# cosmodesi/cosmoprimo

Hardware: AMD Instinct MI355X
Metric: batched FFTLog P(k)->xi(r) transforms/sec (N=2048) (higher is better)
Workload: dtype f64; 1 GPU; config 2: 100000 rows x N_k=2048 per GPU, PowerToCorrelation(ell=0), Np=4096, extrap=0; rows_per_gpu=100000, n_k=2048, padded_size=4096, parallelism=rows sharded over 1 GPU(s), no collective, grid=512, block=256, lds_bytes=69936, rccl_ranks=0

## Files before the change

### cosmoprimo_amd/_lib.py

```python
import ctypes
import os

import numpy as np

_HERE = os.path.dirname(os.path.abspath(__file__))
LIB_PATH = os.path.join(_HERE, 'libcosmoprimo_amd.so')
ABI_VERSION = 4

CP_OK, CP_EINVAL, CP_EUNSUPPORTED, CP_EDEVICE, CP_ENOMEM = range(5)
EXTRAP_CONSTANT, EXTRAP_EDGE, EXTRAP_LOGLOG = range(3)
(KERNEL_BESSEL_J, KERNEL_SPHERICAL_BESSEL_J, KERNEL_TOPHAT, KERNEL_TOPHAT_SQ, KERNEL_GAUSSIAN, KERNEL_GAUSSIAN_SQ) = range(6)
KERNEL_CUSTOM = 100


class FFTlogSpec(ctypes.Structure):
    _fields_ = [('kind', ctypes.c_int), ('param', ctypes.c_double), ('q', ctypes.c_double), ('xy', ctypes.c_double), ('pre_power', ctypes.c_double),
                ('pre_const', ctypes.c_double), ('post_sign', ctypes.c_double)]


_c_double_p = ctypes.POINTER(ctypes.c_double)
_c_int_p = ctypes.POINTER(ctypes.c_int)

SIGNATURES = {
    'cp_abi_version': (ctypes.c_int, []),
# ... 1 lines not shown
    'cp_device_count': (ctypes.c_int, []),
    'cp_loggamma': (ctypes.c_int, [_c_double_p, _c_double_p, ctypes.c_longlong]),
    'cp_gamma': (ctypes.c_int, [_c_double_p, _c_double_p, ctypes.c_longlong]),
    'cp_kernel_eval': (ctypes.c_int, [ctypes.c_int, ctypes.c_double, _c_double_p, _c_double_p, ctypes.c_longlong]),
    'cp_fftlog_padded_size': (ctypes.c_int, [ctypes.c_int, ctypes.c_int]),
    'cp_fftlog_tables': (ctypes.c_int, [ctypes.c_int, ctypes.c_int, _c_double_p, ctypes.POINTER(FFTlogSpec), ctypes.c_int, ctypes.c_int, ctypes.c_int,
                                       _c_double_p, _c_double_p] + [_c_double_p] * 8),
    'cp_fftlog_plan_create': (ctypes.c_int, [ctypes.POINTER(ctypes.c_void_p), ctypes.c_int, ctypes.c_int, ctypes.c_int, _c_double_p,
                                            _c_double_p, _c_double_p, ctypes.c_int]),
    'cp_fftlog_execute': (ctypes.c_int, [ctypes.c_void_p, ctypes.c_void_p, ctypes.c_void_p, ctypes.c_longlong, ctypes.c_int, ctypes.c_double,
                                        ctypes.c_int, ctypes.c_double, ctypes.c_int, ctypes.c_void_p]),
    'cp_fftlog_execute_window': (ctypes.c_int, [ctypes.c_void_p, ctypes.c_void_p, ctypes.c_void_p, ctypes.c_longlong, ctypes.c_int, ctypes.c_double,
                                               ctypes.c_int, ctypes.c_double, ctypes.c_int, ctypes.c_int, ctypes.c_int, ctypes.c_void_p]),
    'cp_fftlog_plan_destroy': (ctypes.c_int, [ctypes.c_void_p]),
    'cp_fftlog_plan_info': (ctypes.c_int, [ctypes.c_void_p, ctypes.c_longlong, _c_int_p, _c_int_p, _c_int_p]),
    'cp_background_distance': (ctypes.c_int, [ctypes.c_longlong, ctypes.c_longlong, ctypes.c_void_p, ctypes.c_int, ctypes.c_void_p, ctypes.c_int,
                                             ctypes.c_void_p, ctypes.c_int, ctypes.c_int, ctypes.c_void_p]),
    'cp_derived_parameters': (ctypes.c_int, [ctypes.c_longlong, ctypes.c_void_p, ctypes.c_void_p, ctypes.c_int, ctypes.c_void_p]),
    'cp_background_knots': (ctypes.c_int, [_c_double_p, ctypes.c_int]),
    'cp_background_init': (ctypes.c_int, [ctypes.c_int]),
    'cp_distance_from_radial': (ctypes.c_int, [ctypes.c_void_p, ctypes.c_void_p, ctypes.c_longlong, ctypes.c_double, ctypes.c_int, ctypes.c_void_p, ctypes.c_int, ctypes.c_void_p]),
    'cp_ncdm_knots': (ctypes.c_int, [_c_double_p, ctypes.c_int]),
    'cp_growth_ode_knots': (ctypes.c_int, [_c_double_p, ctypes.c_int]),
    'cp_growth_ode_tables': (ctypes.c_int, [ctypes.c_longlong, ctypes.c_void_p, ctypes.c_int, ctypes.c_void_p, ctypes.c_int, ctypes.c_void_p, ctypes.c_int,
                                           ctypes.c_void_p]),
    'cp_ncdm_tables': None,
    'cp_background_eval': (ctypes.c_int, [ctypes.c_longlong, ctypes.c_longlong, ctypes.c_void_p, ctypes.c_int, ctypes.c_void_p, ctypes.c_void_p,
                                         ctypes.c_int, ctypes.c_void_p, ctypes.c_int, ctypes.c_int, ctypes.c_void_p]),
    'cp_power_workspace_bytes': (ctypes.c_longlong, [ctypes.c_longlong]),
    'cp_power_eval': (ctypes.c_int, [ctypes.c_int, ctypes.c_int, ctypes.c_longlong, ctypes.c_void_p, ctypes.c_int, ctypes.c_void_p, ctypes.c_void_p,
# ... 265 lines not shown
```

### cosmoprimo_amd/csrc/cp_fftlog.hip

```cpp
#include <hip/hip_runtime.h>

#include <cstring>
#include <new>
#include <vector>

#include "../../include/cosmoprimo_amd.h"
#include "cp_error.h"
#include "cp_fftlog_kernel.h"
#include "cp_fftlog_large.h"
#include "cp_internal.h"

using namespace cpfft;

namespace {

bool find_launcher(int npad, Launcher* out) {
    return find_launcher_g0(npad, out) || find_launcher_g1(npad, out) || find_launcher_g2(npad, out) || find_launcher_g3(npad, out) ||
           find_launcher_g4(npad, out);
}

}

struct cp_fftlog_plan {
    int n, npad, nker, device;
    int in_left, out_left;
    Launcher l;
    int max_grid[VAR_COUNT];
    double* d_pre;
    double* d_post;
    cplx* d_u;
    cplx* d_tw;
    unsigned* d_ticket;
    cp_fftlog_large* large;
};

#define CP_HIP(call)                                                                               \
    do {                                                                                           \
        hipError_t e_ = (call);                                                                    \
        if (e_ != hipSuccess) {                                                                    \
            status = cp::fail(e_ == hipErrorOutOfMemory ? CP_ENOMEM : CP_EDEVICE, "%s: %s", #call, hipGetErrorString(e_)); \
            goto done;                                                                             \
        }                                                                                          \
    } while (0)

bool cp_fftlog_plan_view(const cp_fftlog_plan* p, cp_fftlog_tables_view* out) {
    if (!p || p->large || !out) return false;
    *out = cp_fftlog_tables_view{p->n, p->npad, p->nker, p->device, p->in_left, p->out_left, p->d_pre, p->d_post, p->d_u, p->d_tw};
    return true;
}
// ... 17 lines not shown
    if (npad < n || (npad & (npad - 1)) != 0)
        return cp::fail(CP_EINVAL, "cp_fftlog_plan_create: padded size %d must be a power of two >= n=%d (fftlog.py:149-159)", npad, n);
    Launcher l;
    if (npad > (1 << 24)) return cp::fail(CP_EUNSUPPORTED, "cp_fftlog_plan_create: padded size %d is beyond the supported range (2^24)", npad);
    if ((long long)nker * npad > (1LL << 28))
        return cp::fail(CP_EUNSUPPORTED, "cp_fftlog_plan_create: %d transforms of padded size %d: tables of more than 2^28 entries", nker, npad);
    if (npad > CP_FFTLOG_MAX_NP) {
        cp_fftlog_plan* p = new (std::nothrow) cp_fftlog_plan();
        if (!p) return cp::fail(CP_ENOMEM, "cp_fftlog_plan_create: host allocation failed");
        p->n = n; p->npad = npad; p->nker = nker; p->device = device;
        p->in_left = (npad - n) / 2;
        p->out_left = (npad - n) - (npad - n) / 2;
        p->d_pre = p->d_post = nullptr;
        p->d_u = p->d_tw = nullptr;
        p->d_ticket = nullptr;
        p->large = nullptr;
        cp::DeviceScope scope(device);
        int st = scope.ok() ? cp_fftlog_large_create(&p->large, n, npad, nker, pre, post, u_re_im, device)
                          : cp::fail(CP_EDEVICE, "cp_fftlog_plan_create: cannot select device %d", device);
        if (st != CP_OK) {
            delete p;
            return st;
        }
        *out = p;
        return CP_OK;
    }
    if (!find_launcher(npad, &l))
        return cp::fail(CP_EUNSUPPORTED, "cp_fftlog_plan_create: padded size %d outside the LDS-resident kernel range [4, %d]", npad,
                        CP_FFTLOG_MAX_NP);
    int status = CP_OK;
    cp_fftlog_plan* p = new (std::nothrow) cp_fftlog_plan();
    if (!p) return cp::fail(CP_ENOMEM, "cp_fftlog_plan_create: host allocation failed");
    p->large = nullptr;
    p->n = n;
    p->npad = npad;
    p->nker = nker;
    p->device = device;
    p->in_left = (npad - n) / 2;
    p->out_left = (npad - n) - (npad - n) / 2;
    p->l = l;
    p->d_pre = p->d_post = nullptr;
    p->d_u = p->d_tw = nullptr;
    p->d_ticket = nullptr;
    {
        cp::DeviceScope scope(device);
        std::vector<cplx> tw, u((size_t)nker * npad);
        if (!scope.ok()) {
            status = cp::fail(CP_EDEVICE, "cp_fftlog_plan_create: cannot select device %d", device);
            goto done;
        }
        l.build_tw(tw);
        for (int k = 0; k < nker; ++k) l.build_u(u_re_im + (size_t)k * 2 * (npad / 2 + 1), u.data() + (size_t)k * npad);
        const size_t tbytes = (size_t)nker * npad * sizeof(double);
        CP_HIP(hipMalloc(&p->d_pre, tbytes));
        CP_HIP(hipMalloc(&p->d_post, tbytes));
        CP_HIP(hipMalloc(&p->d_u, u.size() * sizeof(cplx)));
        CP_HIP(hipMalloc(&p->d_tw, tw.size() * sizeof(cplx)));
        CP_HIP(hipMemcpy(p->d_pre, pre, tbytes, hipMemcpyHostToDevice));
        CP_HIP(hipMemcpy(p->d_post, post, tbytes, hipMemcpyHostToDevice));
        CP_HIP(hipMemcpy(p->d_u, u.data(), u.size() * sizeof(cplx), hipMemcpyHostToDevice));
        CP_HIP(hipMemcpy(p->d_tw, tw.data(), tw.size() * sizeof(cplx), hipMemcpyHostToDevice));
        CP_HIP(hipMalloc(&p->d_ticket, CP_CU_SLOTS * sizeof(unsigned)));
        CP_HIP(hipMemset(p->d_ticket, 0, CP_CU_SLOTS * sizeof(unsigned)));
        int ncu = 0;
        CP_HIP(hipDeviceGetAttribute(&ncu, hipDeviceAttributeMultiprocessorCount, device));
        for (int v = 0; v < VAR_COUNT; ++v) {
            p->max_grid[v] = 0;
            if (!l.func[v]) continue;
            const int lds_v = l.lds_bytes + l.lds_extra[v];
            if (lds_v > 64 * 1024) CP_HIP(hipFuncSetAttribute(l.func[v], hipFuncAttributeMaxDynamicSharedMemorySize, lds_v));
            int nblk = 0;
            CP_HIP(hipOccupancyMaxActiveBlocksPerMultiprocessor(&nblk, l.func[v], l.block, lds_v));
            if (nblk < 1) {
                status = cp::fail(CP_EDEVICE, "cp_fftlog_plan_create: kernel variant %d for npad=%d does not fit on a CU", v, npad);
                goto done;
            }
            p->max_grid[v] = nblk * ncu;
        }
// ... 4 lines not shown
        return status;
    }
    *out = p;
    return CP_OK;
}

extern "C" int cp_fftlog_plan_destroy(cp_fftlog_plan* p) {
    if (!p) return CP_OK;
    {
        cp::DeviceScope scope(p->device);
        if (p->d_pre) (void)hipFree(p->d_pre);
        if (p->d_post) (void)hipFree(p->d_post);
        if (p->d_u) (void)hipFree(p->d_u);
        if (p->d_tw) (void)hipFree(p->d_tw);
        if (p->d_ticket) (void)hipFree(p->d_ticket);
        cp_fftlog_large_destroy(p->large);
    }
    delete p;
    return CP_OK;
}

static int grid_for(const cp_fftlog_plan* p, int variant, long long nbatch) {
    const long long npairs = ((nbatch + 1) / 2) * p->nker;
    return (int)(npairs < p->max_grid[variant] ? npairs : p->max_grid[variant]);
}

extern "C" int cp_fftlog_plan_info(const cp_fftlog_plan* p, long long nbatch, int* grid, int* block, int* lds_bytes) {
    if (!p) return cp::fail(CP_EINVAL, "cp_fftlog_plan_info: null plan");
    if (p->large) {
        if (grid) *grid = 0;
        if (block) *block = 0;
        if (lds_bytes) *lds_bytes = 0;
        return CP_OK;
    }
    const int variant = select_variant(p->npad, p->l.p, p->n, 0, 0., 0, 0., 0);
    if (grid) *grid = grid_for(p, variant, nbatch);
    if (block) *block = p->l.block;
    if (lds_bytes) *lds_bytes = p->l.lds_bytes + p->l.lds_extra[variant];
    return CP_OK;
}

static int execute_impl(const cp_fftlog_plan* p, const double* d_in, double* d_out, long long nbatch, int extrap_left, double val_left, int extrap_right,
                        double val_right, int keep_padding, int out_first, int out_count, void* stream) {
    if (!p) return cp::fail(CP_EINVAL, "cp_fftlog_execute: null plan");
    if (nbatch < 0) return cp::fail(CP_EINVAL, "cp_fftlog_execute: negative batch");
    if (nbatch == 0) return CP_OK;
    if (!d_in || !d_out) return cp::fail(CP_EINVAL, "cp_fftlog_execute: null device pointer");
    if (extrap_left < CP_EXTRAP_CONSTANT || extrap_left > CP_EXTRAP_LOGLOG || extrap_right < CP_EXTRAP_CONSTANT || extrap_right > CP_EXTRAP_LOGLOG)
        return cp::fail(CP_EINVAL, "cp_fftlog_execute: unknown extrapolation mode (%d, %d)", extrap_left, extrap_right);
    if (p->large) {
        cp::DeviceScope scope(p->device);
        if (!scope.ok()) return cp::fail(CP_EDEVICE, "cp_fftlog_execute: cannot select device %d", p->device);
        return cp_fftlog_large_execute(p->large, d_in, d_out, nbatch, extrap_left, val_left, extrap_right, val_right, keep_padding,
// ... 20 lines not shown
    A.cu_ticket = p->d_ticket;
    A.out_first = 0;
    A.out_last = A.n_out;
    cp::DeviceScope scope(p->device);
    if (!scope.ok()) return cp::fail(CP_EDEVICE, "cp_fftlog_execute: cannot select device %d", p->device);
    int variant = select_variant(p->npad, p->l.p, p->n, extrap_left, val_left, extrap_right, val_right, keep_padding);
    if (variant == VAR_HALF_ZERO && out_count >= 0 && out_count < A.n_out && p->l.func[VAR_HALF_ZERO_WINDOW]) {
        variant = VAR_HALF_ZERO_WINDOW;
        A.out_first = out_first;
        A.out_last = out_first + out_count;
        A.stream_rows = (double)nbatch * p->nker * ((double)p->n + out_count) * 8. > 512. * 1024. * 1024. ? 3 : 0;
    }
    const int grid = grid_for(p, variant, nbatch);
    if ((long long)p->nker * p->npad >= (1LL << 31) || 2LL * grid * p->npad >= (1LL << 31))
        return cp::fail(CP_EUNSUPPORTED, "cp_fftlog_execute: nker = %d kernels of padded size %d exceed the row-walk range", p->nker, p->npad);
    p->l.launch(variant, A, grid, static_cast<hipStream_t>(stream));
    return cp::launch_status("cp_fftlog_execute");
}

extern "C" int cp_fftlog_execute(const cp_fftlog_plan* p, const double* d_in, double* d_out, long long nbatch, int extrap_left,
                                 double val_left, int extrap_right, double val_right, int keep_padding, void* stream) {
    return execute_impl(p, d_in, d_out, nbatch, extrap_left, val_left, extrap_right, val_right, keep_padding, 0, -1, stream);
}

extern "C" int cp_fftlog_execute_window(const cp_fftlog_plan* p, const double* d_in, double* d_out, long long nbatch, int extrap_left, double val_left,
                                        int extrap_right, double val_right, int keep_padding, int out_first, int out_count, void* stream) {
    if (p) {
        const int n_out = keep_padding ? p->npad : p->n;
        if (out_first < 0 || out_count < 0 || out_first > n_out - out_count)
            return cp::fail(CP_EINVAL, "cp_fftlog_execute_window: columns [%d, %d + %d) are not inside the %d of an output row", out_first, out_first, out_count, n_out);
// ... 4 lines not shown
```

### cosmoprimo_amd/csrc/cp_fftlog_body.h

```cpp
#pragma once
#include <math.h>

#include "cp_fft_core.h"
#if defined(__HIPCC__)
#include "cp_math.h"
#endif

namespace cpfft {

enum { CP_EXTRAP_CONST = 0, CP_EXTRAP_EDGE = 1, CP_EXTRAP_LOG = 2 };

#ifndef CP_INTERPAIR_BARRIER
#define CP_INTERPAIR_BARRIER 0
#endif
#ifndef CP_WAVE_SKEW
#define CP_WAVE_SKEW 1
#endif
#ifndef CP_WAVE_ORDER
#define CP_WAVE_ORDER 0x3210
#endif
#ifndef CP_WIDE_IO
#define CP_WIDE_IO 0
#endif
#ifndef CP_ROW_SCREEN
// ... 21 lines not shown
    long long nbatch;
    int nker;
    int n;
    int in_left;
    int out_off;
    int n_out;
    int ext_l, ext_r;
    double val_l, val_r;
    int stream_rows;
    const double* pre;
    const double* post;
    const cplx* u;
    const cplx* tw;
    int out_first, out_last;
    unsigned* cu_ticket;
#if defined(CP_STAMPS)
    double* val_stamp;
    unsigned long long* bar_log;
    int bar_log_pairs;
#endif
};

template <int NP, int P, int IN_MODE = IN_LOG, int OUT_MODE = OUT_GENERIC>
struct Fftlog {
    using PL = Plan<NP, P>;
    static constexpr int T = PL::T;
    static constexpr int NPASS = PL::NPASS;
    static constexpr int NPH = 2 * NPASS - 1;
    static constexpr int LAST = NPASS - 1;
    static constexpr bool EARLY_TW1 = CP_EARLY_TW1 && NPASS >= 3 && CP_ABLATE == 0;
// ... 407 lines not shown
                const int o = nidx - A.out_off;
                if (o >= 0 && o < A.n_out) {
                    const double f = post[nidx];
                    double ya = x[s].re * f, yb = x[s].im * f;
                    if constexpr (SCREEN) fix_output<1>(fix, &ya, &yb);
                    oa[o] = ya;
                    if (has_b) ob[o] = yb;
                }
            }
        }
    }

    struct State {
        int t0;
        unsigned info_cur, info_nxt;
        cplx w[P];
        cplx wpin[KPIN > 0 ? KPIN : 1];
        double fpre[H], fpost[H];
        double va[H], vb[H];
#if defined(CP_STAMPS)
        unsigned long long fs[8], fs_last;
#endif
    };

    template <int I>
    static CP_HD void load_twiddles(int t, const FftlogArgs& A, cplx* w) {
        Pass<NP, P, I>::template twiddle_load<(I == 0 ? KPIN : 0)>(t, A.tw + PL::tw_offset(I), w);
    }
    template <class ST>
    static CP_HD void merge_pinned(const ST& st, cplx* wl) {
// ... 40 lines not shown
            }
#pragma unroll
            for (int r = 0; r < H; ++r) {
                st.va[r] *= st.fpre[r];
                st.vb[r] *= st.fpre[r];
            }
            unsigned ma = 0, mb = 0;
            thread_max<H>(st.va, st.vb, ma, mb);
            screen_publish(t, lds, ma, mb);
        }
#endif
    }

    static CP_HD void init_state(int t, const FftlogArgs& A, const double* ra, const double* rb, int ker, State& st) {
        st.t0 = pass0_thread(t);
        if constexpr (NPASS > 1) load_twiddles<0>(st.t0, A, st.w);
        if constexpr (KPIN > 0) {
            const cplx* tw0 = A.tw + PL::tw_offset(0);
#pragma unroll
            for (int s = 1; s <= KPIN; ++s) st.wpin[s - 1] = ld_cplx(tw0, (unsigned)st.t0 * 16u, (unsigned)(s * T) * 16u);
        }
        if constexpr (HALF_IN) {
            load_factors_half(st.t0, A, ker, st);
            if constexpr (ROWS_FROM_MEMORY) prefetch_rows(st.t0, ra, rb, st.va, st.vb, A.stream_rows);
        }
    }

    template <int PHN>
    static CP_HD void load_tables_for(int t, int t0, const FftlogArgs& A, int ker, cplx* w) {
        if constexpr (PHN == LAST) {
// ... 33 lines not shown
        if constexpr (NPASS == 1) {
            load_input(t0, t, A, ra, rb, has_b, pre, lds, st.info_cur, x);
            Pass<NP, P, 0>::butterflies(x);
            load_u(t0, A, ker, st.w);
            mul_w(st.w, x);
            Pass<NP, P, 0>::butterflies(x);
            store_output(t0, A, oa, ob, has_b, post, st.info_cur, x);
        } else if constexpr (PH == 0) {
            if constexpr (HALF_IN) {
#if defined(__HIP_DEVICE_COMPILE__)
                if constexpr (SCREEN_AHEAD) st.info_cur = gate(st.info_nxt);
#endif
                load_input_half(t0, t, A, ra, rb, has_b, pre, lds, st, x);
                CP_SCHED_FENCE();
                if constexpr (ROWS_FROM_MEMORY) prefetch_rows(t0, nra, nrb, st.va, st.vb, A.stream_rows);
                CP_SCHED_FENCE();
            } else {
                load_input(t0, t, A, ra, rb, has_b, pre, lds, st.info_cur, x);
            }
            if constexpr (KPIN > 0) {
                cplx wl[P];
                merge_pinned(st, wl);
                Pass<NP, P, 0>::template butterflies_store<ZERO_PADDED_IN, true>(t0, wl, lds, x);
            } else {
                Pass<NP, P, 0>::template butterflies_store<ZERO_PADDED_IN, true>(t0, st.w, lds, x);
            }
            load_tables_for<1>(t, t0, A, ker, st.w);
            if constexpr (EARLY_TW1) Pass<NP, P, 1>::twiddle_load_lds(t, lds_tw<1>(lds), st.w);
        } else if constexpr (PH < LAST) {
            constexpr int I = (PH < LAST) ? PH : 0;
// ... 60 lines not shown
```

### cosmoprimo_amd/csrc/cp_fftlog_dispatch.h

```cpp
#pragma once

#ifdef CP_FFTLOG_ONLY
#define CP_FFTLOG_SIZES(X) X(CP_FFTLOG_ONLY, 16)
#else
#define CP_FFTLOG_SIZES(X) \
    X(4, 4)                \
    X(8, 8)                \
    X(16, 16)              \
    X(32, 16)              \
    X(64, 16)              \
    X(128, 16)             \
    X(256, 16)             \
    X(512, 16)             \
    X(1024, 16)            \
    X(2048, 16)            \
    X(4096, 16)            \
    X(8192, 16)
#endif

#define CP_FFTLOG_MAX_NP 8192

enum { VAR_GENERIC = 0, VAR_LOG = 1, VAR_HALF = 2, VAR_HALF_ZERO = 3, VAR_HALF_ZERO_WINDOW = 4, VAR_COUNT = 5 };

#define CP_FFTLOG_HALF_MIN_NP 512

inline int select_variant(int np, int p, int n, int ext_l, double val_l, int ext_r, double val_r, int keep_padding) {
    if (ext_l == 2 || ext_r == 2) return VAR_LOG;
    if ((p == 16 || p == 8) && np >= CP_FFTLOG_HALF_MIN_NP && 2 * n == np && !keep_padding) {
        if (ext_l == 0 && ext_r == 0 && val_l == 0. && val_r == 0.) return VAR_HALF_ZERO;
        return VAR_HALF;
    }
    return VAR_GENERIC;
}
```

### cosmoprimo_amd/csrc/cp_fftlog_kernel.h

```cpp
#pragma once
#include <hip/hip_runtime.h>

#include <vector>

#include "cp_fftlog_body.h"
#include "cp_fftlog_dispatch.h"
#include "cp_fftlog_tables.h"

namespace cpfft {

struct Launcher {
    const void* func[VAR_COUNT];
    void (*launch)(int variant, const FftlogArgs&, int grid, hipStream_t stream);
    int np, p, block, lds_bytes;
    int lds_extra[VAR_COUNT];
    void (*build_tw)(std::vector<cplx>&);
    void (*build_u)(const double*, cplx*);
};

bool find_launcher_g0(int npad, Launcher* out);
bool find_launcher_g1(int npad, Launcher* out);
bool find_launcher_g2(int npad, Launcher* out);
bool find_launcher_g3(int npad, Launcher* out);
bool find_launcher_g4(int npad, Launcher* out);

#if defined(__HIPCC__)
#if defined(CP_STAMPS)
#define CP_STAMP_DECL , unsigned long long *cp_stamp_acc, unsigned long long *cp_bar_log
#define CP_STAMP_ARG , cp_stamp_acc, cp_bar_log
#else
#define CP_STAMP_DECL
#define CP_STAMP_ARG
#endif
template <int NP, int P, int IM, int OM>
constexpr bool balances_cu();
template <int NP, int P, int IM, int OM>
constexpr bool skews_waves() {
    using F = Fftlog<NP, P, IM, OM>;
    if constexpr (CP_WAVE_SKEW > 0 && F::NPH == 5 && F::T == 256) {
        return balances_cu<NP, P, IM, OM>() && F::template barrier_free_after<1>() && F::template barrier_free_after<2>();
    }
    return false;
}

template <int NP, int P, int IM, int OM, int PH>
__device__ __forceinline__ void run_phases(int t, const FftlogArgs& A, const double* ra, const double* rb, double* oa, double* ob, bool has_b,
                                           int ker, cplx* lds, const double* nra, const double* nrb, int nxt_ker,
                                           typename Fftlog<NP, P, IM, OM>::State& st CP_STAMP_DECL) {
    using F = Fftlog<NP, P, IM, OM>;
#if defined(CP_STAMPS)
    const unsigned long long s0 = cp_stamp();
#endif
    F::template phase<PH>(t, A, ra, rb, oa, ob, has_b, ker, lds, nra, nrb, nxt_ker, st);
#if defined(CP_STAMPS)
    const unsigned long long s1 = cp_stamp();
    cp_stamp_acc[2 * PH] += s1 - s0;
#endif
    if constexpr (PH + 1 < F::NPH) {
        if constexpr (F::template barrier_free_after<PH>()) {
            asm volatile("" ::: "memory");
        } else if (!(CP_ABLATE & 2)) {
            __syncthreads();
            if constexpr (PH == 0 && skews_waves<NP, P, IM, OM>()) {
                const int w = __builtin_amdgcn_readfirstlane((int)(threadIdx.x >> 6));
                for (int i = 0, n = (int)((CP_WAVE_ORDER >> (4 * w)) & 0xf) * CP_WAVE_SKEW; i < n; ++i) __builtin_amdgcn_s_sleep(1);
                asm volatile("" ::: "memory");
            }
        }
#if defined(CP_STAMPS)
        const unsigned long long s2 = cp_stamp();
        cp_stamp_acc[2 * PH + 1] += s2 - s1;
        if constexpr (!F::template barrier_free_after<PH>()) {
            if (cp_bar_log && (threadIdx.x & 63) == 0) cp_bar_log[PH == 0 ? 0 : 1] = s2;
        }
#endif
        run_phases<NP, P, IM, OM, PH + 1>(t, A, ra, rb, oa, ob, has_b, ker, lds, nra, nrb, nxt_ker, st CP_STAMP_ARG);
    }
}

struct PairRows {
    long long in_off, out_off;
    int ker;
    int has_b;
};

struct PairWalk {
    PairRows cur;
    long long p, p_last_q;
    unsigned in_step, out_step;
    unsigned in_b, out_b;
    int dker, odd;
// ... 38 lines not shown
}

#define CP_CU_SLOTS 4096
#if defined(__HIPCC__)
__device__ __forceinline__ unsigned cp_cu_id() {
    unsigned hw, xcc;
    asm volatile("s_getreg_b32 %0, hwreg(HW_REG_HW_ID)" : "=s"(hw));
    asm volatile("s_getreg_b32 %0, hwreg(HW_REG_XCC_ID)" : "=s"(xcc));
    return ((xcc & 0xfu) << 8) | ((hw >> 8) & 0xffu);
}
#endif

#ifndef CP_BALANCE_PCT
#define CP_BALANCE_PCT 65
#endif
#define CP_BALANCE_LDS 16
template <int NP, int P, int IM, int OM>
constexpr bool balances_cu() {
    return CP_BALANCE_PCT > 0 && CP_ABLATE == 0 && NP == 4096 && P == 16 && IM == IN_HALF_ZERO && OM == OUT_HALF;
}

#ifndef CP_WAVES_PER_SIMD
#define CP_WAVES_PER_SIMD 2
#endif
template <int NP, int P, int IM, int OM>
__global__ __launch_bounds__(NP / P, CP_WAVES_PER_SIMD) void fftlog_kernel(const FftlogArgs A) {
    extern __shared__ __attribute__((aligned(4096))) char smem[];
    cplx* lds = reinterpret_cast<cplx*>(smem);
    using F = Fftlog<NP, P, IM, OM>;
    const int t = threadIdx.x;
    const long long nhalf = (A.nbatch + 1) / 2;
    const long long npairs = nhalf * A.nker;
    typename F::State st;
    long long p = blockIdx.x;
    if (p >= npairs) return;
    PairWalk walk = pair_walk_begin(A, p, gridDim.x);
    PairRows cur = walk.cur;
    {
        const double* ra = A.in + cur.in_off;
        F::init_state(t, A, ra, ra + (cur.has_b ? walk.in_b : 0u), cur.ker, st);
    }
    constexpr bool BALANCE = balances_cu<NP, P, IM, OM>();
    if constexpr (BALANCE) {
        if (threadIdx.x == 0) reinterpret_cast<unsigned*>(smem + F::LDS_BYTES)[0] = atomicAdd(A.cu_ticket + cp_cu_id(), 1u) & 1u;
    }
    if constexpr (F::NPASS > 1) {
        F::fill_lds_tables(t, A, lds);
        F::screen_prefetched(t, st.t0, A, cur.ker, lds, st);
        __syncthreads();
        if constexpr (F::SCREEN_AHEAD) st.info_nxt = F::screen_collect(lds);
    }
    int bal_odd = 0, bal_switch = -1, bal_k = 0;
    if constexpr (BALANCE) {
        bal_odd = __builtin_amdgcn_readfirstlane((int)reinterpret_cast<unsigned*>(smem + F::LDS_BYTES)[0]);
        const int mine = (int)((npairs - blockIdx.x + gridDim.x - 1) / gridDim.x);
        const int first = (mine * CP_BALANCE_PCT + 50) / 100;
        bal_switch = bal_odd ? first : mine - first;
        if (bal_odd) __builtin_amdgcn_s_setprio(1);
    }
    __builtin_amdgcn_s_waitcnt(0x0F70);
#if defined(CP_START_STAGGER)
    for (int i = 0, n = (int)((blockIdx.x / CP_STAGGER_DIV) % CP_STAGGER_MOD) * CP_START_STAGGER; i < n; ++i) __builtin_amdgcn_s_sleep(64);
#endif
#if defined(CP_STAMPS)
    unsigned long long cp_stamp_acc[2 * F::NPH] = {0};
    for (int i = 0; i < 8; ++i) st.fs[i] = 0;
    const unsigned long long cp_t_begin = cp_stamp();
    unsigned long long* cp_bar_log = nullptr;
    if (A.bar_log && __builtin_amdgcn_readfirstlane(threadIdx.x >> 6) == 0) {
        cp_bar_log = A.bar_log + (size_t)blockIdx.x * (2 + 2 * (size_t)A.bar_log_pairs);
        if (threadIdx.x == 0) cp_bar_log[0] = cp_cu_id(), cp_bar_log[1] = cp_t_begin;
        cp_bar_log += 2;
    }
#endif
    for (;;) {
        if constexpr (BALANCE) {
            if (bal_k++ == bal_switch) {
                if (bal_odd) __builtin_amdgcn_s_setprio(0);
                else __builtin_amdgcn_s_setprio(1);
            }
        }
        const bool more = walk.p + gridDim.x < npairs;
        if (more) pair_walk_next(A, walk, gridDim.x);
        const PairRows nxt = walk.cur;
        const double* ra = A.in + cur.in_off;
        double* oa = A.out + cur.out_off;
        const double* nra = A.in + nxt.in_off;
        run_phases<NP, P, IM, OM, 0>(t, A, ra, ra + (cur.has_b ? walk.in_b : 0u), oa, oa + (cur.has_b ? walk.out_b : 0u), cur.has_b, cur.ker,
                                     lds, nra, nra + (nxt.has_b ? walk.in_b : 0u), nxt.ker, st CP_STAMP_ARG);
        if (!more) break;
#if defined(CP_STAMPS)
        const unsigned long long sb = cp_stamp();
#endif
#if defined(CP_STAMPS)
        cp_stamp_acc[2 * F::NPH - 1] += cp_stamp() - sb;
        if (cp_bar_log) cp_bar_log += 2;
#endif
        cur = nxt;
    }
#if defined(CP_STAMPS)
    if ((threadIdx.x & 63) == 0) {
        unsigned long long* dst = reinterpret_cast<unsigned long long*>(const_cast<double*>(A.val_stamp)) +
                                  ((size_t)blockIdx.x * (NP / P / 64) + threadIdx.x / 64) * (2 * F::NPH + 1 + 8);
        for (int i = 0; i < 2 * F::NPH; ++i) dst[i] = cp_stamp_acc[i];
        dst[2 * F::NPH] = cp_stamp() - cp_t_begin;
        unsigned hw;
        asm volatile("s_getreg_b32 %0, hwreg(HW_REG_HW_ID)" : "=s"(hw));
        st.fs[0] = (hw >> 4) & 3u;
        for (int i = 0; i < 8; ++i) dst[2 * F::NPH + 1 + i] = st.fs[i];
    }
#endif
}

template <int NP, int P>
constexpr bool has_half() {
    return (P == 16 || P == 8) && NP >= CP_FFTLOG_HALF_MIN_NP;
}

template <int NP, int P>
void launch_impl(int variant, const FftlogArgs& A, int grid, hipStream_t stream) {
    constexpr int T = Plan<NP, P>::T;
    constexpr int lds = Fftlog<NP, P>::LDS_BYTES;
    if constexpr (has_half<NP, P>()) {
        if (variant == VAR_HALF_ZERO) {
            constexpr int extra = balances_cu<NP, P, IN_HALF_ZERO, OUT_HALF>() ? CP_BALANCE_LDS : 0;
            hipLaunchKernelGGL((fftlog_kernel<NP, P, IN_HALF_ZERO, OUT_HALF>), dim3(grid), dim3(T), lds + extra, stream, A);
            return;
        }
        if (variant == VAR_HALF) {
            hipLaunchKernelGGL((fftlog_kernel<NP, P, IN_HALF, OUT_HALF>), dim3(grid), dim3(T), lds, stream, A);
            return;
        }
        if (variant == VAR_HALF_ZERO_WINDOW) {
            hipLaunchKernelGGL((fftlog_kernel<NP, P, IN_HALF_ZERO, OUT_HALF_WINDOW>), dim3(grid), dim3(T), lds, stream, A);
            return;
        }
    }
    if (variant == VAR_LOG)
        hipLaunchKernelGGL((fftlog_kernel<NP, P, IN_LOG, OUT_GENERIC>), dim3(grid), dim3(T), lds, stream, A);
    else
        hipLaunchKernelGGL((fftlog_kernel<NP, P, IN_GENERIC, OUT_GENERIC>), dim3(grid), dim3(T), lds, stream, A);
}

template <int NP, int P>
Launcher make_launcher() {
    Launcher l;
    for (int v = 0; v < VAR_COUNT; ++v) l.func[v] = nullptr, l.lds_extra[v] = 0;
    l.func[VAR_GENERIC] = reinterpret_cast<const void*>(&fftlog_kernel<NP, P, IN_GENERIC, OUT_GENERIC>);
    l.func[VAR_LOG] = reinterpret_cast<const void*>(&fftlog_kernel<NP, P, IN_LOG, OUT_GENERIC>);
    if constexpr (has_half<NP, P>()) {
        l.func[VAR_HALF] = reinterpret_cast<const void*>(&fftlog_kernel<NP, P, IN_HALF, OUT_HALF>);
        l.func[VAR_HALF_ZERO] = reinterpret_cast<const void*>(&fftlog_kernel<NP, P, IN_HALF_ZERO, OUT_HALF>);
        if (balances_cu<NP, P, IN_HALF_ZERO, OUT_HALF>()) l.lds_extra[VAR_HALF_ZERO] = CP_BALANCE_LDS;
        l.func[VAR_HALF_ZERO_WINDOW] = reinterpret_cast<const void*>(&fftlog_kernel<NP, P, IN_HALF_ZERO, OUT_HALF_WINDOW>);
    }
    l.launch = &launch_impl<NP, P>;
    l.np = NP;
    l.p = P;
    l.block = Plan<NP, P>::T;
    l.lds_bytes = Fftlog<NP, P>::LDS_BYTES;
    l.build_tw = &build_twiddles<NP, P>;
    l.build_u = &build_u_layout<NP, P>;
    return l;
}
#endif

}
```

### include/cosmoprimo_amd.h

```cpp
#ifndef COSMOPRIMO_AMD_H
#define COSMOPRIMO_AMD_H

#ifdef __cplusplus
extern "C" {
#endif

#define CP_ABI_VERSION 4

enum cp_status {
    CP_OK = 0,
    CP_EINVAL = 1,
    CP_EUNSUPPORTED = 2,
    CP_EDEVICE = 3,
    CP_ENOMEM = 4
};

enum cp_extrap { CP_EXTRAP_CONSTANT = 0, CP_EXTRAP_EDGE = 1, CP_EXTRAP_LOGLOG = 2 };

enum cp_kernel {
    CP_KERNEL_BESSEL_J = 0,
    CP_KERNEL_SPHERICAL_BESSEL_J = 1,
    CP_KERNEL_TOPHAT = 2,
    CP_KERNEL_TOPHAT_SQ = 3,
    CP_KERNEL_GAUSSIAN = 4,
// ... 21 lines not shown
int cp_fftlog_padded_size(int n, int minfolds);
int cp_fftlog_tables(int n, int nker, const double* x, const cp_fftlog_spec* spec, int minfolds, int lowring, int check_level,
                     const double* u_custom, const double* lowring_custom, double* delta, double* lnxy, double* y, double* padded_x,
                     double* padded_y, double* pre, double* post, double* u);

typedef struct cp_fftlog_plan cp_fftlog_plan;

int cp_fftlog_plan_create(cp_fftlog_plan** plan, int n, int npad, int nker, const double* pre, const double* post,
                          const double* u_re_im, int device);
int cp_fftlog_execute(const cp_fftlog_plan* plan, const double* d_in, double* d_out, long long nbatch, int extrap_left,
                      double val_left, int extrap_right, double val_right, int keep_padding, void* stream);
int cp_fftlog_execute_window(const cp_fftlog_plan* plan, const double* d_in, double* d_out, long long nbatch, int extrap_left, double val_left,
                             int extrap_right, double val_right, int keep_padding, int out_first, int out_count, void* stream);
int cp_fftlog_plan_destroy(cp_fftlog_plan* plan);
int cp_fftlog_plan_info(const cp_fftlog_plan* plan, long long nbatch, int* grid, int* block, int* lds_bytes);

enum cp_bg_param {
    CP_BG_H = 0, CP_BG_OMEGA_CDM = 1 , CP_BG_OMEGA_B = 2, CP_BG_OMEGA_K = 3, CP_BG_T_CMB = 4,
    CP_BG_N_UR = 5, CP_BG_W0_FLD = 6, CP_BG_WA_FLD = 7, CP_BG_NPARAMS = 8
};
enum cp_bg_kind {
    CP_BG_COMOVING_RADIAL = 0,
    CP_BG_COMOVING_TRANSVERSE = 1,
    CP_BG_ANGULAR_DIAMETER = 2,
    CP_BG_LUMINOSITY = 3,
    CP_BG_EFUNC = 4,
    CP_BG_HUBBLE = 5,
    CP_BG_GROWTH_CPT = 6,
    CP_BG_GROWTH_RATE = 7,
    CP_BG_RHO_CRIT = 8,
// ... 289 lines not shown
```

Before: 106.2 million transforms/s.

## Replace static pair striding with dynamic atomic work claiming in headline FFTLog kernel

Adds a claim variant of the headline NP=4096 half-zero kernel in which persistent blocks take their next row pair from a per-stream global atomic counter instead of a fixed grid stride. The claim is issued early, during the input phase, and passed through LDS near the last barrier so it stays off the critical path. The last block to leave resets the counter. The aim is to smooth load imbalance across CUs at the tail of the batch, at the cost of one atomic per pair, extra host-side mutex and stream-capture checks per launch, and per-stream claim slots.

```diff
diff --git a/cosmoprimo_amd/_lib.py b/cosmoprimo_amd/_lib.py
--- a/cosmoprimo_amd/_lib.py
+++ b/cosmoprimo_amd/_lib.py
@@ -39,6 +39,8 @@
                                                ctypes.c_int, ctypes.c_double, ctypes.c_int, ctypes.c_int, ctypes.c_int, ctypes.c_void_p]),
     'cp_fftlog_plan_destroy': (ctypes.c_int, [ctypes.c_void_p]),
     'cp_fftlog_plan_info': (ctypes.c_int, [ctypes.c_void_p, ctypes.c_longlong, _c_int_p, _c_int_p, _c_int_p]),
+    'cp_fftlog_plan_set_claims': (ctypes.c_int, [ctypes.c_void_p, ctypes.c_int]),
+    'cp_fftlog_plan_claims': (ctypes.c_int, [ctypes.c_void_p, ctypes.POINTER(ctypes.c_uint), ctypes.c_int, _c_int_p]),
     'cp_background_distance': (ctypes.c_int, [ctypes.c_longlong, ctypes.c_longlong, ctypes.c_void_p, ctypes.c_int, ctypes.c_void_p, ctypes.c_int,
                                              ctypes.c_void_p, ctypes.c_int, ctypes.c_int, ctypes.c_void_p]),
     'cp_derived_parameters': (ctypes.c_int, [ctypes.c_longlong, ctypes.c_void_p, ctypes.c_void_p, ctypes.c_int, ctypes.c_void_p]),
diff --git a/cosmoprimo_amd/csrc/cp_fftlog.hip b/cosmoprimo_amd/csrc/cp_fftlog.hip
--- a/cosmoprimo_amd/csrc/cp_fftlog.hip
+++ b/cosmoprimo_amd/csrc/cp_fftlog.hip
@@ -1,6 +1,7 @@
 #include <hip/hip_runtime.h>
 
 #include <cstring>
+#include <mutex>
 #include <new>
 #include <vector>
 
@@ -21,6 +22,7 @@
 
 }
 
+#define CP_CLAIM_SLOTS 64
 struct cp_fftlog_plan {
     int n, npad, nker, device;
     int in_left, out_left;
@@ -31,8 +33,32 @@
     cplx* d_u;
     cplx* d_tw;
     unsigned* d_ticket;
+    unsigned* d_claims;
+    mutable std::mutex claim_lock;
+    mutable hipStream_t claim_stream[CP_CLAIM_SLOTS];
+    mutable int claim_streams;
+    int claims_on;
     cp_fftlog_large* large;
 };
+
+static unsigned* claim_slot(const cp_fftlog_plan* p, hipStream_t stream) {
+    if (!p->d_claims || stream == hipStreamPerThread) return nullptr;
+    hipStreamCaptureStatus capture = hipStreamCaptureStatusNone;
+    if (hipStreamIsCapturing(stream, &capture) != hipSuccess) {
+        (void)hipGetLastError();
+        return nullptr;
+    }
+    if (capture != hipStreamCaptureStatusNone) return nullptr;
+    std::lock_guard<std::mutex> guard(p->claim_lock);
+    if (!p->claims_on) return nullptr;
+    int i = 0;
+    while (i < p->claim_streams && p->claim_stream[i] != stream) ++i;
+    if (i == p->claim_streams) {
+        if (i == CP_CLAIM_SLOTS) return nullptr;
+        p->claim_stream[p->claim_streams++] = stream;
+    }
+    return p->d_claims + 2 * i;
+}
 
 #define CP_HIP(call)                                                                               \
     do {                                                                                           \
@@ -80,6 +106,9 @@
         p->d_pre = p->d_post = nullptr;
         p->d_u = p->d_tw = nullptr;
         p->d_ticket = nullptr;
+        p->d_claims = nullptr;
+        p->claim_streams = 0;
+        p->claims_on = 0;
         p->large = nullptr;
         cp::DeviceScope scope(device);
         int st = scope.ok() ? cp_fftlog_large_create(&p->large, n, npad, nker, pre, post, u_re_im, device)
@@ -108,6 +137,9 @@
     p->d_pre = p->d_post = nullptr;
     p->d_u = p->d_tw = nullptr;
     p->d_ticket = nullptr;
+    p->d_claims = nullptr;
+    p->claim_streams = 0;
+    p->claims_on = 1;
     {
         cp::DeviceScope scope(device);
         std::vector<cplx> tw, u((size_t)nker * npad);
@@ -128,6 +160,8 @@
         CP_HIP(hipMemcpy(p->d_tw, tw.data(), tw.size() * sizeof(cplx), hipMemcpyHostToDevice));
         CP_HIP(hipMalloc(&p->d_ticket, CP_CU_SLOTS * sizeof(unsigned)));
         CP_HIP(hipMemset(p->d_ticket, 0, CP_CU_SLOTS * sizeof(unsigned)));
+        CP_HIP(hipMalloc(&p->d_claims, CP_CLAIM_SLOTS * 2 * sizeof(unsigned)));
+        CP_HIP(hipMemset(p->d_claims, 0, CP_CLAIM_SLOTS * 2 * sizeof(unsigned)));
         int ncu = 0;
         CP_HIP(hipDeviceGetAttribute(&ncu, hipDeviceAttributeMultiprocessorCount, device));
         for (int v = 0; v < VAR_COUNT; ++v) {
@@ -162,6 +196,7 @@
         if (p->d_u) (void)hipFree(p->d_u);
         if (p->d_tw) (void)hipFree(p->d_tw);
         if (p->d_ticket) (void)hipFree(p->d_ticket);
+        if (p->d_claims) (void)hipFree(p->d_claims);
         cp_fftlog_large_destroy(p->large);
     }
     delete p;
@@ -185,6 +220,26 @@
     if (grid) *grid = grid_for(p, variant, nbatch);
     if (block) *block = p->l.block;
     if (lds_bytes) *lds_bytes = p->l.lds_bytes + p->l.lds_extra[variant];
+    return CP_OK;
+}
+
+extern "C" int cp_fftlog_plan_set_claims(cp_fftlog_plan* p, int on) {
+    if (!p) return cp::fail(CP_EINVAL, "cp_fftlog_plan_set_claims: null plan");
+    std::lock_guard<std::mutex> guard(p->claim_lock);
+    p->claims_on = on != 0;
+    return CP_OK;
+}
+
+extern "C" int cp_fftlog_plan_claims(const cp_fftlog_plan* p, unsigned* host, int capacity, int* words) {
+    if (!p) return cp::fail(CP_EINVAL, "cp_fftlog_plan_claims: null plan");
+    const int n = p->d_claims ? 2 * CP_CLAIM_SLOTS : 0;
+    if (words) *words = n;
+    if (host && capacity > 0 && n > 0) {
+        cp::DeviceScope scope(p->device);
+        if (!scope.ok()) return cp::fail(CP_EDEVICE, "cp_fftlog_plan_claims: cannot select device %d", p->device);
+        const hipError_t e = hipMemcpy(host, p->d_claims, (size_t)(capacity < n ? capacity : n) * sizeof(unsigned), hipMemcpyDeviceToHost);
+        if (e != hipSuccess) return cp::fail(CP_EDEVICE, "cp_fftlog_plan_claims: %s", hipGetErrorString(e));
+    }
     return CP_OK;
 }
 
@@ -235,6 +290,11 @@
     const int grid = grid_for(p, variant, nbatch);
     if ((long long)p->nker * p->npad >= (1LL << 31) || 2LL * grid * p->npad >= (1LL << 31))
         return cp::fail(CP_EUNSUPPORTED, "cp_fftlog_execute: nker = %d kernels of padded size %d exceed the row-walk range", p->nker, p->npad);
+    A.claims = nullptr;
+    if (variant == VAR_HALF_ZERO && p->l.func[VAR_HALF_ZERO_CLAIM] && p->nker == 1 && (nbatch + 1) / 2 + 3LL * grid < (1LL << 32)) {
+        A.claims = claim_slot(p, static_cast<hipStream_t>(stream));
+        if (A.claims) variant = VAR_HALF_ZERO_CLAIM;
+    }
     p->l.launch(variant, A, grid, static_cast<hipStream_t>(stream));
     return cp::launch_status("cp_fftlog_execute");
 }
diff --git a/cosmoprimo_amd/csrc/cp_fftlog_body.h b/cosmoprimo_amd/csrc/cp_fftlog_body.h
--- a/cosmoprimo_amd/csrc/cp_fftlog_body.h
+++ b/cosmoprimo_amd/csrc/cp_fftlog_body.h
@@ -59,6 +59,7 @@
     const cplx* tw;
     int out_first, out_last;
     unsigned* cu_ticket;
+    unsigned* claims;
 #if defined(CP_STAMPS)
     double* val_stamp;
     unsigned long long* bar_log;
@@ -496,6 +497,8 @@
     struct State {
         int t0;
         unsigned info_cur, info_nxt;
+        bool claim_on;
+        unsigned claim, claim_nxt;
         cplx w[P];
         cplx wpin[KPIN > 0 ? KPIN : 1];
         double fpre[H], fpost[H];
@@ -566,6 +569,8 @@
 
     static CP_HD void init_state(int t, const FftlogArgs& A, const double* ra, const double* rb, int ker, State& st) {
         st.t0 = pass0_thread(t);
+        st.claim_on = false;
+        st.claim = st.claim_nxt = 0u;
         if constexpr (NPASS > 1) load_twiddles<0>(st.t0, A, st.w);
         if constexpr (KPIN > 0) {
             const cplx* tw0 = A.tw + PL::tw_offset(0);
@@ -629,6 +634,15 @@
                 load_input_half(t0, t, A, ra, rb, has_b, pre, lds, st, x);
                 CP_SCHED_FENCE();
                 if constexpr (ROWS_FROM_MEMORY) prefetch_rows(t0, nra, nrb, st.va, st.vb, A.stream_rows);
+#if defined(__HIP_DEVICE_COMPILE__)
+                if constexpr (IN_MODE == IN_HALF_ZERO && OUT_MODE == OUT_HALF) {
+                    if (st.claim_on && t == 0) {
+                        unsigned zero = 0;
+                        asm volatile("" : "+v"(zero));
+                        st.claim = atomicAdd(A.claims + zero, 1u);
+                    }
+                }
+#endif
                 CP_SCHED_FENCE();
             } else {
                 load_input(t0, t, A, ra, rb, has_b, pre, lds, st.info_cur, x);
diff --git a/cosmoprimo_amd/csrc/cp_fftlog_dispatch.h b/cosmoprimo_amd/csrc/cp_fftlog_dispatch.h
--- a/cosmoprimo_amd/csrc/cp_fftlog_dispatch.h
+++ b/cosmoprimo_amd/csrc/cp_fftlog_dispatch.h
@@ -20,7 +20,7 @@
 
 #define CP_FFTLOG_MAX_NP 8192
 
-enum { VAR_GENERIC = 0, VAR_LOG = 1, VAR_HALF = 2, VAR_HALF_ZERO = 3, VAR_HALF_ZERO_WINDOW = 4, VAR_COUNT = 5 };
+enum { VAR_GENERIC = 0, VAR_LOG = 1, VAR_HALF = 2, VAR_HALF_ZERO = 3, VAR_HALF_ZERO_WINDOW = 4, VAR_HALF_ZERO_CLAIM = 5, VAR_COUNT = 6 };
 
 #define CP_FFTLOG_HALF_MIN_NP 512
 
diff --git a/cosmoprimo_amd/csrc/cp_fftlog_kernel.h b/cosmoprimo_amd/csrc/cp_fftlog_kernel.h
--- a/cosmoprimo_amd/csrc/cp_fftlog_kernel.h
+++ b/cosmoprimo_amd/csrc/cp_fftlog_kernel.h
@@ -26,24 +26,32 @@
 
 #if defined(__HIPCC__)
 #if defined(CP_STAMPS)
+#define CP_BAR_LOG_HEAD 3
 #define CP_STAMP_DECL , unsigned long long *cp_stamp_acc, unsigned long long *cp_bar_log
 #define CP_STAMP_ARG , cp_stamp_acc, cp_bar_log
 #else
 #define CP_STAMP_DECL
 #define CP_STAMP_ARG
 #endif
-template <int NP, int P, int IM, int OM>
-constexpr bool balances_cu();
+#define CP_HEADLINE_LDS 16
+template <class F>
+__device__ __forceinline__ unsigned* cp_claim_word(cplx* lds) {
+    return reinterpret_cast<unsigned*>(reinterpret_cast<char*>(lds) + F::LDS_BYTES) + 1;
+}
+template <int NP, int P, int IM, int OM>
+constexpr bool is_headline();
+template <int NP, int P, int IM, int OM>
+constexpr bool claims_pairs();
 template <int NP, int P, int IM, int OM>
 constexpr bool skews_waves() {
     using F = Fftlog<NP, P, IM, OM>;
     if constexpr (CP_WAVE_SKEW > 0 && F::NPH == 5 && F::T == 256) {
-        return balances_cu<NP, P, IM, OM>() && F::template barrier_free_after<1>() && F::template barrier_free_after<2>();
+        return is_headline<NP, P, IM, OM>() && F::template barrier_free_after<1>() && F::template barrier_free_after<2>();
     }
     return false;
 }
 
-template <int NP, int P, int IM, int OM, int PH>
+template <int NP, int P, int IM, int OM, int PH, bool CLAIM = false>
 __device__ __forceinline__ void run_phases(int t, const FftlogArgs& A, const double* ra, const double* rb, double* oa, double* ob, bool has_b,
                                            int ker, cplx* lds, const double* nra, const double* nrb, int nxt_ker,
                                            typename Fftlog<NP, P, IM, OM>::State& st CP_STAMP_DECL) {
@@ -60,7 +68,13 @@
         if constexpr (F::template barrier_free_after<PH>()) {
             asm volatile("" ::: "memory");
         } else if (!(CP_ABLATE & 2)) {
+            if constexpr (PH == F::NPH - 2 && CLAIM) {
+                if (st.claim_on && threadIdx.x == 0) cp_claim_word<F>(lds)[0] = st.claim;
+            }
             __syncthreads();
+            if constexpr (PH == F::NPH - 2 && CLAIM) {
+                if (st.claim_on) st.claim_nxt = (unsigned)__builtin_amdgcn_readfirstlane((int)cp_claim_word<F>(lds)[0]);
+            }
             if constexpr (PH == 0 && skews_waves<NP, P, IM, OM>()) {
                 const int w = __builtin_amdgcn_readfirstlane((int)(threadIdx.x >> 6));
                 for (int i = 0, n = (int)((CP_WAVE_ORDER >> (4 * w)) & 0xf) * CP_WAVE_SKEW; i < n; ++i) __builtin_amdgcn_s_sleep(1);
@@ -74,7 +88,7 @@
             if (cp_bar_log && (threadIdx.x & 63) == 0) cp_bar_log[PH == 0 ? 0 : 1] = s2;
         }
 #endif
-        run_phases<NP, P, IM, OM, PH + 1>(t, A, ra, rb, oa, ob, has_b, ker, lds, nra, nrb, nxt_ker, st CP_STAMP_ARG);
+        run_phases<NP, P, IM, OM, PH + 1, CLAIM>(t, A, ra, rb, oa, ob, has_b, ker, lds, nra, nrb, nxt_ker, st CP_STAMP_ARG);
     }
 }
 
@@ -143,17 +157,44 @@
 #ifndef CP_BALANCE_PCT
 #define CP_BALANCE_PCT 65
 #endif
-#define CP_BALANCE_LDS 16
+template <int NP, int P, int IM, int OM>
+constexpr bool is_headline() {
+    return CP_ABLATE == 0 && NP == 4096 && P == 16 && IM == IN_HALF_ZERO && OM == OUT_HALF;
+}
 template <int NP, int P, int IM, int OM>
 constexpr bool balances_cu() {
-    return CP_BALANCE_PCT > 0 && CP_ABLATE == 0 && NP == 4096 && P == 16 && IM == IN_HALF_ZERO && OM == OUT_HALF;
-}
+    return CP_BALANCE_PCT > 0 && is_headline<NP, P, IM, OM>();
+}
+
+#ifndef CP_CLAIM_PAIRS
+#define CP_CLAIM_PAIRS 1
+#endif
+#ifndef CP_CLAIM_TRADE
+#define CP_CLAIM_TRADE 1
+#endif
+template <int NP, int P, int IM, int OM>
+constexpr bool claims_pairs() {
+    return CP_CLAIM_PAIRS && is_headline<NP, P, IM, OM>() && Fftlog<NP, P, IM, OM>::NPASS > 1;
+}
+#if defined(__HIPCC__)
+__device__ __forceinline__ void cp_claims_leave(unsigned* claims) {
+    if (threadIdx.x == 0) {
+        __threadfence();
+        const unsigned old = atomicAdd(claims + 1, 1u);
+        if (old == gridDim.x - 1) {
+            __hip_atomic_store(claims, 0u, __ATOMIC_RELAXED, __HIP_MEMORY_SCOPE_AGENT);
+            __hip_atomic_store(claims + 1, 0u, __ATOMIC_RELAXED, __HIP_MEMORY_SCOPE_AGENT);
+        }
+    }
+}
+#endif
 
 #ifndef CP_WAVES_PER_SIMD
 #define CP_WAVES_PER_SIMD 2
 #endif
-template <int NP, int P, int IM, int OM>
+template <int NP, int P, int IM, int OM, bool CLAIM = false>
 __global__ __launch_bounds__(NP / P, CP_WAVES_PER_SIMD) void fftlog_kernel(const FftlogArgs A) {
+    static_assert(!CLAIM || claims_pairs<NP, P, IM, OM>(), "only the headline variant claims its pairs");
     extern __shared__ __attribute__((aligned(4096))) char smem[];
     cplx* lds = reinterpret_cast<cplx*>(smem);
     using F = Fftlog<NP, P, IM, OM>;
@@ -162,27 +203,35 @@
     const long long npairs = nhalf * A.nker;
     typename F::State st;
     long long p = blockIdx.x;
-    if (p >= npairs) return;
+    if (p >= npairs) {
+        if constexpr (CLAIM) cp_claims_leave(A.claims);
+        return;
+    }
     PairWalk walk = pair_walk_begin(A, p, gridDim.x);
     PairRows cur = walk.cur;
     {
         const double* ra = A.in + cur.in_off;
         F::init_state(t, A, ra, ra + (cur.has_b ? walk.in_b : 0u), cur.ker, st);
     }
-    constexpr bool BALANCE = balances_cu<NP, P, IM, OM>();
+    constexpr bool BALANCE = balances_cu<NP, P, IM, OM>() && (!CLAIM || CP_CLAIM_TRADE);
     if constexpr (BALANCE) {
         if (threadIdx.x == 0) reinterpret_cast<unsigned*>(smem + F::LDS_BYTES)[0] = atomicAdd(A.cu_ticket + cp_cu_id(), 1u) & 1u;
+    }
+    unsigned claim_nxt = 0;
+    if constexpr (CLAIM) {
+        if (threadIdx.x == 0) cp_claim_word<F>(lds)[0] = gridDim.x + atomicAdd(A.claims, 1u);
     }
     if constexpr (F::NPASS > 1) {
         F::fill_lds_tables(t, A, lds);
         F::screen_prefetched(t, st.t0, A, cur.ker, lds, st);
         __syncthreads();
         if constexpr (F::SCREEN_AHEAD) st.info_nxt = F::screen_collect(lds);
+        if constexpr (CLAIM) claim_nxt = (unsigned)__builtin_amdgcn_readfirstlane((int)cp_claim_word<F>(lds)[0]);
     }
     int bal_odd = 0, bal_switch = -1, bal_k = 0;
     if constexpr (BALANCE) {
         bal_odd = __builtin_amdgcn_readfirstlane((int)reinterpret_cast<unsigned*>(smem + F::LDS_BYTES)[0]);
-        const int mine = (int)((npairs - blockIdx.x + gridDim.x - 1) / gridDim.x);
+        const int mine = (int)((npairs - (CLAIM ? 0 : blockIdx.x) + gridDim.x - 1) / gridDim.x);
         const int first = (mine * CP_BALANCE_PCT + 50) / 100;
         bal_switch = bal_odd ? first : mine - first;
         if (bal_odd) __builtin_amdgcn_s_setprio(1);
@@ -197,10 +246,11 @@
     const unsigned long long cp_t_begin = cp_stamp();
     unsigned long long* cp_bar_log = nullptr;
     if (A.bar_log && __builtin_amdgcn_readfirstlane(threadIdx.x >> 6) == 0) {
-        cp_bar_log = A.bar_log + (size_t)blockIdx.x * (2 + 2 * (size_t)A.bar_log_pairs);
+        cp_bar_log = A.bar_log + (size_t)blockIdx.x * (CP_BAR_LOG_HEAD + 2 * (size_t)A.bar_log_pairs);
         if (threadIdx.x == 0) cp_bar_log[0] = cp_cu_id(), cp_bar_log[1] = cp_t_begin;
-        cp_bar_log += 2;
-    }
+        cp_bar_log += CP_BAR_LOG_HEAD;
+    }
+    int cp_pairs_run = 0;
 #endif
     for (;;) {
         if constexpr (BALANCE) {
@@ -209,13 +259,25 @@
                 else __builtin_amdgcn_s_setprio(1);
             }
         }
-        const bool more = walk.p + gridDim.x < npairs;
-        if (more) pair_walk_next(A, walk, gridDim.x);
-        const PairRows nxt = walk.cur;
+        bool more;
+        PairRows nxt = cur;
+        if constexpr (CLAIM) {
+            more = claim_nxt < npairs;
+            if (more) {
+                nxt.in_off = 2ll * claim_nxt * A.n;
+                nxt.out_off = 2ll * claim_nxt * A.n_out;
+                nxt.has_b = !((A.nbatch & 1) && claim_nxt == npairs - 1);
+            }
+            st.claim_on = more;
+        } else {
+            more = walk.p + gridDim.x < npairs;
+            if (more) pair_walk_next(A, walk, gridDim.x);
+            nxt = walk.cur;
+        }
         const double* ra = A.in + cur.in_off;
         double* oa = A.out + cur.out_off;
         const double* nra = A.in + nxt.in_off;
-        run_phases<NP, P, IM, OM, 0>(t, A, ra, ra + (cur.has_b ? walk.in_b : 0u), oa, oa + (cur.has_b ? walk.out_b : 0u), cur.has_b, cur.ker,
+        run_phases<NP, P, IM, OM, 0, CLAIM>(t, A, ra, ra + (cur.has_b ? walk.in_b : 0u), oa, oa + (cur.has_b ? walk.out_b : 0u), cur.has_b, cur.ker,
                                      lds, nra, nra + (nxt.has_b ? walk.in_b : 0u), nxt.ker, st CP_STAMP_ARG);
         if (!more) break;
 #if defined(CP_STAMPS)
@@ -223,11 +285,15 @@
 #endif
 #if defined(CP_STAMPS)
         cp_stamp_acc[2 * F::NPH - 1] += cp_stamp() - sb;
-        if (cp_bar_log) cp_bar_log += 2;
+        if (cp_bar_log && ++cp_pairs_run < A.bar_log_pairs) cp_bar_log += 2;
 #endif
         cur = nxt;
-    }
-#if defined(CP_STAMPS)
+        if constexpr (CLAIM) claim_nxt = st.claim_nxt + gridDim.x;
+    }
+    if constexpr (CLAIM) cp_claims_leave(A.claims);
+#if defined(CP_STAMPS)
+    if (A.bar_log && threadIdx.x == 0)
+        A.bar_log[(size_t)blockIdx.x * (CP_BAR_LOG_HEAD + 2 * (size_t)A.bar_log_pairs) + 2] = (unsigned long long)cp_pairs_run + 1;
     if ((threadIdx.x & 63) == 0) {
         unsigned long long* dst = reinterpret_cast<unsigned long long*>(const_cast<double*>(A.val_stamp)) +
                                   ((size_t)blockIdx.x * (NP / P / 64) + threadIdx.x / 64) * (2 * F::NPH + 1 + 8);
@@ -252,9 +318,15 @@
     constexpr int lds = Fftlog<NP, P>::LDS_BYTES;
     if constexpr (has_half<NP, P>()) {
         if (variant == VAR_HALF_ZERO) {
-            constexpr int extra = balances_cu<NP, P, IN_HALF_ZERO, OUT_HALF>() ? CP_BALANCE_LDS : 0;
+            constexpr int extra = is_headline<NP, P, IN_HALF_ZERO, OUT_HALF>() ? CP_HEADLINE_LDS : 0;
             hipLaunchKernelGGL((fftlog_kernel<NP, P, IN_HALF_ZERO, OUT_HALF>), dim3(grid), dim3(T), lds + extra, stream, A);
             return;
+        }
+        if constexpr (claims_pairs<NP, P, IN_HALF_ZERO, OUT_HALF>()) {
+            if (variant == VAR_HALF_ZERO_CLAIM) {
+                hipLaunchKernelGGL((fftlog_kernel<NP, P, IN_HALF_ZERO, OUT_HALF, true>), dim3(grid), dim3(T), lds + CP_HEADLINE_LDS, stream, A);
+                return;
+            }
         }
         if (variant == VAR_HALF) {
             hipLaunchKernelGGL((fftlog_kernel<NP, P, IN_HALF, OUT_HALF>), dim3(grid), dim3(T), lds, stream, A);
@@ -280,7 +352,11 @@
     if constexpr (has_half<NP, P>()) {
         l.func[VAR_HALF] = reinterpret_cast<const void*>(&fftlog_kernel<NP, P, IN_HALF, OUT_HALF>);
         l.func[VAR_HALF_ZERO] = reinterpret_cast<const void*>(&fftlog_kernel<NP, P, IN_HALF_ZERO, OUT_HALF>);
-        if (balances_cu<NP, P, IN_HALF_ZERO, OUT_HALF>()) l.lds_extra[VAR_HALF_ZERO] = CP_BALANCE_LDS;
+        if (is_headline<NP, P, IN_HALF_ZERO, OUT_HALF>()) l.lds_extra[VAR_HALF_ZERO] = CP_HEADLINE_LDS;
+        if constexpr (claims_pairs<NP, P, IN_HALF_ZERO, OUT_HALF>()) {
+            l.func[VAR_HALF_ZERO_CLAIM] = reinterpret_cast<const void*>(&fftlog_kernel<NP, P, IN_HALF_ZERO, OUT_HALF, true>);
+            l.lds_extra[VAR_HALF_ZERO_CLAIM] = CP_HEADLINE_LDS;
+        }
         l.func[VAR_HALF_ZERO_WINDOW] = reinterpret_cast<const void*>(&fftlog_kernel<NP, P, IN_HALF_ZERO, OUT_HALF_WINDOW>);
     }
     l.launch = &launch_impl<NP, P>;
diff --git a/include/cosmoprimo_amd.h b/include/cosmoprimo_amd.h
--- a/include/cosmoprimo_amd.h
+++ b/include/cosmoprimo_amd.h
@@ -59,6 +59,8 @@
                              int extrap_right, double val_right, int keep_padding, int out_first, int out_count, void* stream);
 int cp_fftlog_plan_destroy(cp_fftlog_plan* plan);
 int cp_fftlog_plan_info(const cp_fftlog_plan* plan, long long nbatch, int* grid, int* block, int* lds_bytes);
+int cp_fftlog_plan_set_claims(cp_fftlog_plan* plan, int on);
+int cp_fftlog_plan_claims(const cp_fftlog_plan* plan, unsigned* host, int capacity, int* words);
 
 enum cp_bg_param {
     CP_BG_H = 0, CP_BG_OMEGA_CDM = 1 , CP_BG_OMEGA_B = 2, CP_BG_OMEGA_K = 3, CP_BG_T_CMB = 4,
```

New measurement: 105.7 million transforms/s. About the same (-0.5%).
